# canghaiyang/Erasure_Coding_Test

Measured on AMD Instinct MI355X. Metric: GiB/s device-resident RS encode+decode, RS(10,4) 4 MiB shards, 1/2/4/8 GPU, higher is better.
Workload: dtype u8

## Files before the change

### erasure_coding_test_amd/build.py

```python
from __future__ import annotations

import hashlib
import os
import re
import shutil
import subprocess
import sys

PKG = os.path.dirname(os.path.abspath(__file__))
ROOT = os.path.dirname(PKG)
CSRC = os.path.join(PKG, "csrc")
LIB = os.path.join(PKG, "lib")
OBJ = os.path.join(PKG, "build", "obj")
INCLUDE = os.path.join(ROOT, "include")

ARCH = os.environ.get("ECGPU_ARCH", "gfx950")
HIPCC = os.environ.get("HIPCC", shutil.which("hipcc") or "/opt/rocm/bin/hipcc")
CXX = os.environ.get("CXX", "g++")

HOST_SRCS = ["gf_host.cpp", "matrix_host.cpp", "planner.cpp", "schedule_host.cpp", "capi_host.cpp", "contract_host.cpp", "knobs.cpp",
             "cpu_fallback.cpp", "cpu_exec.cpp"]
HIP_UNITS = [(f, f + ".o", []) for f in ("ecgpu_runtime.hip", "plans.hip", "devices.hip", "contexts.hip",
                                           "host_memory.hip", "dispatch_w8.hip", "dispatch_wide.hip", "accum.hip",
                                           "pipeline.hip", "packets.hip", "scrub.hip")] + [
# ... 2 lines not shown
DROPIN_SRCS = ["jerasure_dropin.cpp", "jerasure_surface.cpp"]

CXXFLAGS = ["-O2", "-std=c++17", "-fPIC", "-Wall", "-Wextra", "-Wno-unused-parameter", f"-I{INCLUDE}", f"-I{CSRC}"]
HIPFLAGS = ["-O3", "-std=c++17", "-fPIC", "-fvisibility=hidden", "-Wall", "-Wextra", "-Wno-unused-parameter", f"--offload-arch={ARCH}", f"-I{INCLUDE}", f"-I{CSRC}",
            "-Wno-unused-result"]


def _run(cmd):
    print("  " + " ".join(cmd), flush=True)
    subprocess.run(cmd, check=True)


def _run_parallel(cmds):
    from concurrent.futures import ThreadPoolExecutor
    if not cmds:
        return
    workers = max(1, min(len(cmds), int(os.environ.get("MAX_JOBS", "0")) or (os.cpu_count() or 1), 8))
    with ThreadPoolExecutor(workers) as ex:
        for f in [ex.submit(_run, c) for c in cmds]:
            f.result()


KERNEL_FAMILIES = {
    "kernels": (["gf_device.hpp", "gf_kernels_w8.hpp", "gf_spec.hip", "gf_spec.hpp", "dispatch_w8.hip"],
                ["ECGPU_CAP", "ECGPU_BLOCKS_PER_CU", "ECGPU_KERNEL", "ECGPU_NT"]),
    "wide": (["gf_device.hpp", "gf_kernels_wide.hpp", "wide_spec.hip", "wide_spec.hpp", "dispatch_wide.hip"],
             ["ECGPU_WIDE", "ECGPU_NIB16", "ECGPU_WIDE_UNITS", "ECGPU_WIDE_PIPE", "ECGPU_WIDE16_BPCU",
              "ECGPU_WIDE16_UNITS"]),
    "packets": (["gf_device.hpp", "gf_kernels_packets.hpp", "packets.hip"], ["ECGPU_PACKET"]),
    "scrub": (["gf_device.hpp", "scrub_kernels.hpp", "scrub_spec.hip", "scrub_spec.hpp", "scrub.hip"],
              ["ECGPU_CAP", "ECGPU_BLOCKS_PER_CU", "ECGPU_SCRUB_LATE"]),
}


def knob_rows(names) -> list:
    with open(os.path.join(CSRC, "knobs.cpp")) as f:
        lines = f.read().splitlines()
    return [ln.strip() for n in names for ln in lines if ln.strip().startswith('{"%s",' % n)]


def _digest(parts, files) -> str:
    h = hashlib.sha256()
    for p in parts:
        h.update(p.encode())
        h.update(b"\0")
    for f in files:
        h.update(os.path.basename(f).encode())
# ... 146 lines not shown
```

### erasure_coding_test_amd/csrc/diag_kernels.hip

```cpp
#include <hip/hip_runtime.h>

#include <cstdlib>

#include "diag_kernels_w8.hpp"

using ecgpu::dev::ApplyArgs;
using ecgpu::dev::u32x4;
using KernelFn = void (*)(ApplyArgs);

namespace {

__device__ __forceinline__ void sink(const ApplyArgs& a, int s, int64_t col, const u32x4& acc) {
  if (acc.x == 0x9E3779B9u && acc.y == 0x7F4A7C15u && acc.z == 0x85EBCA6Bu && acc.w == 0xC2B2AE35u)
    ecgpu::dev::store16(a.dst[int64_t(s) * a.dst_stride], col, acc, 1);
}

template <int K, int R>
__global__ __launch_bounds__(256) void diag_xor_mix(ApplyArgs a) {
  const int64_t col = int64_t(blockIdx.x) * 256 + threadIdx.x;
  if (col >= a.nvec) return;
  const int s = blockIdx.y;
  const uint8_t* const* sp = a.src + int64_t(s) * a.src_stride;
  uint8_t* dp[R];
#pragma unroll
  for (int r = 0; r < R; ++r) dp[r] = a.dst[int64_t(s) * a.dst_stride + r];
  u32x4 x[K];
#pragma unroll
// ... 108 lines not shown
KernelFn pick_mode(int mode) {
  switch (mode) {
    case 0: return &ecgpu::dev::gf_apply_perm<K, R, V, 0>;
    case 1: return &ecgpu::dev::gf_apply_perm<K, R, V, 1>;
    case 2: return &ecgpu::dev::gf_apply_perm<K, R, V, 2>;
    default: return &ecgpu::dev::gf_apply_perm<K, R, V, 3>;
  }
}
template <int K, int R>
KernelFn pick_vec(int vec, int mode) {
  switch (vec) {
    case 1: return pick_mode<K, R, 1>(mode);
    case 2: return pick_mode<K, R, 2>(mode);
    default: return pick_mode<K, R, 4>(mode);
  }
}
}

extern "C" __attribute__((visibility("default"))) int ecgpu_diag_launch(
    int variant, int K, int R, int vec, int mode, const void* qtab, const void* ntab, const void* src_tab,
    void* dst_tab, int stripes, long long size, unsigned long long unit_mask, unsigned long long zero_mask, int nt,
    void* stream, const void* ptab) {
  KernelFn fn = nullptr;
  if (variant == 0) {
    if (K == 10 && R == 4) fn = pick_vec<10, 4>(vec, mode);
    if (K == 10 && R == 1) fn = pick_vec<10, 1>(vec, mode);
  } else if (variant == 1) {
    using ecgpu::dev::diag_copy;
    KernelFn c1[4] = {&diag_copy<1, 0>, &diag_copy<1, 1>, &diag_copy<1, 2>, &diag_copy<1, 3>};
    KernelFn c2[4] = {&diag_copy<2, 0>, &diag_copy<2, 1>, &diag_copy<2, 2>, &diag_copy<2, 3>};
    KernelFn c4[4] = {&diag_copy<4, 0>, &diag_copy<4, 1>, &diag_copy<4, 2>, &diag_copy<4, 3>};
    fn = (vec == 1 ? c1 : vec == 2 ? c2 : c4)[mode & 3];
  } else if (variant == 3) {
    if (K == 10 && R == 4) fn = mode == 3 ? &ecgpu::dev::gf_apply_perm_stream<10, 4, 3>
                                          : &ecgpu::dev::gf_apply_perm_stream<10, 4, 2>;
    if (K == 10 && R == 1) fn = mode == 3 ? &ecgpu::dev::gf_apply_perm_stream<10, 1, 3>
                                          : &ecgpu::dev::gf_apply_perm_stream<10, 1, 2>;
  } else if (variant == 4 || variant == 5) {
    vec = 1;
    if (K == 10 && R == 4)
      fn = mode == 0 ? &ecgpu::dev::gf_apply<10, 4, 0> : mode == 1 ? &ecgpu::dev::gf_apply<10, 4, 1>
                                                        : &ecgpu::dev::gf_apply<10, 4, 3>;
    if (K == 10 && R == 1)
      fn = mode == 4 ? &ecgpu::dev::gf_apply<10, 1, 4> : &ecgpu::dev::gf_apply<10, 1, 0>;
  } else if (variant == 6) {
    vec = 1;
    if (K == 10 && R == 4) fn = &ecgpu::dev::gf_apply_occ8<10, 4, 3>;
    if (K == 10 && R == 1) fn = mode == 4 ? &ecgpu::dev::gf_apply_occ8<10, 1, 4> : &ecgpu::dev::gf_apply_occ8<10, 1, 0>;
  } else if (variant == 7) {
    const bool occ8 = (vec & 2) != 0;
    if (K == 10 && R == 4)
      fn = occ8 ? &ecgpu::dev::gf_apply_occ8<10, 4, 3> : &ecgpu::dev::gf_apply<10, 4, 3>;
    if (K == 10 && R == 1)
      fn = mode == 4 ? (occ8 ? &ecgpu::dev::gf_apply_occ8<10, 1, 4> : &ecgpu::dev::gf_apply<10, 1, 4>)
                     : (occ8 ? &ecgpu::dev::gf_apply_occ8<10, 1, 0> : &ecgpu::dev::gf_apply<10, 1, 0>);
  } else if (variant == 8) {
    if (K == 10 && R == 4)
      fn = vec == 1 ? &ecgpu::dev::gf_apply<10, 4, 3>
                    : vec == 2 ? &ecgpu::dev::gf_apply_vec<10, 4, 3, 2> : &ecgpu::dev::gf_apply_vec<10, 4, 3, 4>;
    if (K == 10 && R == 1)
      fn = vec == 1 ? &ecgpu::dev::gf_apply<10, 1, 4>
                    : vec == 2 ? &ecgpu::dev::gf_apply_vec<10, 1, 4, 2> : &ecgpu::dev::gf_apply_vec<10, 1, 4, 4>;
  } else if (variant == 9) {
    vec = 1;
    if (K == 1 && R == 1) fn = &ecgpu::dev::gf_apply_perm<1, 1, 1, 3>;
    if (K == 2 && R == 2) fn = &ecgpu::dev::gf_apply_perm<2, 2, 1, 3>;
    if (K == 4 && R == 4) fn = &ecgpu::dev::gf_apply_perm<4, 4, 1, 3>;
    if (K == 7 && R == 7) fn = &ecgpu::dev::gf_apply_perm<7, 7, 1, 3>;
    if (K == 10 && R == 4) fn = &ecgpu::dev::gf_apply_perm<10, 4, 1, 3>;
    if (K == 10 && R == 1) fn = &ecgpu::dev::gf_apply_perm<10, 1, 1, 3>;
    if (K == 13 && R == 1) fn = &ecgpu::dev::gf_apply_perm<13, 1, 1, 3>;
    if (K == 4 && R == 1) fn = &ecgpu::dev::gf_apply_perm<4, 1, 1, 3>;
    if (K == 1 && R == 4) fn = &ecgpu::dev::gf_apply_perm<1, 4, 1, 3>;
    if (K == 2 && R == 1) fn = &ecgpu::dev::gf_apply_perm<2, 1, 1, 3>;
  } else if (variant == 10) {
    vec = 1;
    if (K == 10 && R == 4) fn = &ecgpu::dev::gf_apply_2bit<10, 4, 3>;
    if (K == 10 && R == 1) fn = mode == 4 ? &ecgpu::dev::gf_apply_2bit<10, 1, 4> : &ecgpu::dev::gf_apply_2bit<10, 1, 0>;
  } else if (variant == 11) {
    vec = 1;
    if (K == 1) fn = nt ? &diag_read_regs<1, 1> : &diag_read_regs<1, 0>;
    if (K == 4) fn = nt ? &diag_read_regs<4, 1> : &diag_read_regs<4, 0>;
    if (K == 10) fn = nt ? &diag_read_regs<10, 1> : &diag_read_regs<10, 0>;
    if (K == 14) fn = nt ? &diag_read_regs<14, 1> : &diag_read_regs<14, 0>;
  } else if (variant == 13 || variant == 14) {
    using namespace ecgpu::dev;
    const int ntb = vec;
    vec = 1;
#define ECGPU_PICK(KK, RR, UU)                                                                              \
  (variant == 13 ? (ntb == 0 ? &gf_apply<KK, RR, UU, 0> : ntb == 1 ? &gf_apply<KK, RR, UU, 1>         \
                    : ntb == 2 ? &gf_apply<KK, RR, UU, 2> : &gf_apply<KK, RR, UU, 3>)                 \
                 : (ntb == 0 ? &gf_apply_dma<KK, RR, UU, 0> : ntb == 1 ? &gf_apply_dma<KK, RR, UU, 1> \
                    : ntb == 2 ? &gf_apply_dma<KK, RR, UU, 2> : &gf_apply_dma<KK, RR, UU, 3>))
    if (K == 10 && R == 4) fn = mode == 0 ? ECGPU_PICK(10, 4, 0) : ECGPU_PICK(10, 4, 3);
    if (K == 10 && R == 1) fn = mode == 4 ? ECGPU_PICK(10, 1, 4) : ECGPU_PICK(10, 1, 0);
    if (K == 6 && R == 3) fn = ECGPU_PICK(6, 3, 3);
#undef ECGPU_PICK
  } else if (variant == 12) {
    vec = 1;
    if (K == 1) fn = nt ? &diag_read_glds<1, 1> : &diag_read_glds<1, 0>;
    if (K == 4) fn = nt ? &diag_read_glds<4, 1> : &diag_read_glds<4, 0>;
    if (K == 10) fn = nt ? &diag_read_glds<10, 1> : &diag_read_glds<10, 0>;
    if (K == 14) fn = nt ? &diag_read_glds<14, 1> : &diag_read_glds<14, 0>;
  } else if (variant == 15) {
    const int lp = vec;
    vec = 1;
    if (K == 10 && R == 4) fn = pick_pol<10, 4, 3>(lp, mode);
    if (K == 10 && R == 1) fn = pick_pol<10, 1, 4>(lp, mode);
  } else if (variant == 16) {
    vec = 1;
    if (K == 10 && R == 4) fn = &diag_xor_mix<10, 4>;
    if (K == 10 && R == 1) fn = &diag_xor_mix<10, 1>;
    if (K == 6 && R == 3) fn = &diag_xor_mix<6, 3>;
    if (K == 12 && R == 4) fn = &diag_xor_mix<12, 4>;
    if (K == 4 && R == 2) fn = &diag_xor_mix<4, 2>;
  } else if (variant == 2) {
    vec = 1;
    if (K == 10 && R == 4) fn = &ecgpu::dev::gf_apply_lds<10, 4>;
    if (K == 10 && R == 1) fn = &ecgpu::dev::gf_apply_lds<10, 1>;
  }
  if (!fn) return -2;
  ApplyArgs a{};
  a.qtab = static_cast<const ecgpu::dev::u32x4*>(qtab);
  a.ntab = static_cast<const uint8_t*>(ntab);
  a.ptab = static_cast<const uint32_t*>(ptab);
  a.src = static_cast<const uint8_t* const*>(src_tab);
  a.dst = static_cast<uint8_t* const*>(dst_tab);
  a.nvec = size / 16;
  a.size = size;
  a.byte0 = a.nvec * 16;
  a.unit_mask = unit_mask;
  a.zero_mask = zero_mask;
  a.src_stride = variant == 1 ? 1 : K;
  a.dst_stride = variant == 1 ? 1 : R;
  a.row0 = 0;
  a.K = K;
  a.R = R;
  a.nt = nt;
  const long long per_block = 256LL * (variant == 0 || variant == 1 || variant == 8 ? vec : 1);
  dim3 grid(unsigned((a.nvec + per_block - 1) / per_block), unsigned(stripes));
  if (variant == 3) grid = dim3(unsigned(vec), unsigned(stripes));
  if (variant == 7) {
    a.stripe_fast = vec & 1;
    grid = a.stripe_fast ? dim3(unsigned(stripes), unsigned((a.nvec + 255) / 256))
                         : dim3(unsigned((a.nvec + 255) / 256), unsigned(stripes));
  }
  if (variant == 5) {
    a.stripe_fast = 1;
    grid = dim3(unsigned(stripes), unsigned((a.nvec + 255) / 256));
  }
  void* args[] = {&a};
  const char* lds_env = std::getenv("ECGPU_DIAG_LDS");
  const unsigned lds = lds_env ? unsigned(std::atoi(lds_env)) : 0u;
  if (lds > 65536u && lds <= 163840u &&
      hipFuncSetAttribute(reinterpret_cast<const void*>(fn), hipFuncAttributeMaxDynamicSharedMemorySize, int(lds)) !=
          hipSuccess)
    return -3;
  return hipLaunchKernel(reinterpret_cast<const void*>(fn), grid, dim3(256), args, lds,
                         static_cast<hipStream_t>(stream)) == hipSuccess ? 0 : -3;
}
```

### erasure_coding_test_amd/csrc/diag_kernels_w8.hpp

```cpp
#pragma once
#include "gf_kernels.hpp"

namespace ecgpu {
namespace dev {

__device__ __forceinline__ u32x4 load16(const uint8_t* p, int64_t col, int nt) {
  const gu32x4* a = (const gu32x4*)p + col;
  return nt ? __builtin_nontemporal_load(a) : *a;
}

__device__ __forceinline__ void store16(uint8_t* p, int64_t col, const u32x4& v, int nt) {
  gu32x4* a = (gu32x4*)p + col;
  if (nt)
    __builtin_nontemporal_store(v, a);
  else
    *a = v;
}

__device__ __forceinline__ uint32_t mac_word(uint32_t acc, const u32x4& q, uint32_t x) {
  const uint32_t s0 = x & kLo2, s1 = (x >> 2) & kLo2, s2 = (x >> 4) & kLo2, s3 = (x >> 6) & kLo2;
  return xor3(acc, xor3(perm_lookup(q.x, s0), perm_lookup(q.y, s1), perm_lookup(q.z, s2)), perm_lookup(q.w, s3));
}

__device__ __forceinline__ uint32_t mul3(const uint32_t* __restrict__ t, const Sel3& s) {
// ... 202 lines not shown
  if (col >= a.nvec) return;
  const int w = __builtin_amdgcn_readfirstlane(int(threadIdx.x) >> 6);
  const int lane = threadIdx.x & 63;
  const uint8_t* const* sp = a.src + int64_t(s) * a.src_stride;
  const uint8_t* src[K];
#pragma unroll
  for (int j = 0; j < K; ++j) src[j] = sp[j];
  uint8_t* dp[R];
#pragma unroll
  for (int r = 0; r < R; ++r) dp[r] = a.dst[int64_t(s) * a.dst_stride + a.row0 + r];
#pragma unroll
  for (int j = 0; j < K; ++j)
    __builtin_amdgcn_global_load_lds((const __attribute__((address_space(1))) void*)(src[j] + col * 16),
                                     (__attribute__((address_space(3))) void*)&stage[w][j][0], 16, 0,
                                     (NT & 1) ? 2 : 0);
  asm volatile("s_waitcnt vmcnt(0)" ::: "memory");
  u32x4 x[K];
#pragma unroll
  for (int j = 0; j < K; ++j) x[j] = stage[w][j][lane];
  combine_store<K, R, UNITS, (NT >> 1)>(a, x, dp, col);
}

template <int K, int R, int UNITS>
__global__ __launch_bounds__(kBlock, 8) void gf_apply_occ8(ApplyArgs a) {
  gf_apply_body<K, R, UNITS>(a);
}

template <int K, int R, int MODE>
__global__ __launch_bounds__(kBlock) void gf_apply_perm_stream(ApplyArgs a) {
  __shared__ u32x4 lq[R * K];
  for (int i = threadIdx.x; i < R * K; i += kBlock) lq[i] = a.qtab[i];
  __syncthreads();
  const int s = blockIdx.y;
  const int64_t steps_total = (a.nvec + kBlock - 1) / kBlock;
  const int64_t steps_per_block = (steps_total + gridDim.x - 1) / gridDim.x;
  const int64_t step0 = int64_t(blockIdx.x) * steps_per_block;
  const int64_t step_end = step0 + steps_per_block < steps_total ? step0 + steps_per_block : steps_total;
  if (step0 >= step_end) return;
  const uint8_t* const* sp = a.src + int64_t(s) * a.src_stride;
  uint8_t* dp[R];
#pragma unroll
  for (int r = 0; r < R; ++r) dp[r] = a.dst[int64_t(s) * a.dst_stride + a.row0 + r];
  const uint8_t* src[K];
#pragma unroll
  for (int j = 0; j < K; ++j) src[j] = sp[j];

  u32x4 cur[K], nxt[K];
  int64_t col = step0 * kBlock + threadIdx.x;
// ... 57 lines not shown
```

### erasure_coding_test_amd/csrc/dispatch_w8.hip

```cpp
#include <hip/hip_runtime.h>

#include <algorithm>
#include <atomic>
#include <cstdint>
#include <cstring>
#include <mutex>
#include <string>
#include <utility>
#include <vector>

#include "ecgpu.h"
#include "gf_host.hpp"
#include "gf_kernels_w8.hpp"
#include "knobs.hpp"
#include "runtime.hpp"
#include "gf_spec.hpp"

using namespace ecgpu;
using namespace ecgpu::rt;
using dev::ApplyArgs;
using dev::u32x4;

namespace ecgpu {
namespace dev {

static __global__ __launch_bounds__(kBlock) void gf_apply_bytes(ApplyArgs a) {
  const int64_t x = a.byte0 + int64_t(blockIdx.x) * kBlock + threadIdx.x;
  if (x >= a.size) return;
  const int s = blockIdx.y;
  const uint8_t* const* sp = a.src + int64_t(s) * a.src_stride;
  uint8_t* const* dp = a.dst + int64_t(s) * a.dst_stride + a.row0;
  uint32_t acc[kMaxRows] = {0u, 0u, 0u, 0u};
  for (int j = 0; j < a.K; ++j) {
    const uint32_t v = sp[j][x];
    const uint32_t s0 = v & 3u, s1 = (v >> 2) & 3u, s2 = (v >> 4) & 3u, s3 = v >> 6;
    for (int r = 0; r < a.R; ++r) acc[r] ^= gf_mul_perm(a.qtab[r * a.K + j], s0, s1, s2, s3);
  }
// ... 11 lines not shown
    for (int j = 0; j < K; ++j) {
      const bool one = coef[size_t(r0 + r) * K + j] == 1;
      all &= one;
      if (j == 0) col0 &= one;
      if (r == 0) row0 &= one;
    }
  if (all) return 4;
  return (col0 ? 1 : 0) | (row0 ? 2 : 0);
}

KernelFn generic_fn(int R) {
  switch (R) {
    case 1: return &dev::gf_apply_perm_generic<1>;
    case 2: return &dev::gf_apply_perm_generic<2>;
    case 3: return &dev::gf_apply_perm_generic<3>;
    default: return &dev::gf_apply_perm_generic<4>;
  }
}


constexpr int kCapMaxBlocks = 4;
constexpr int kMinWavesPerSimd = 4;
static_assert(kMinWavesPerSimd >= kCapMaxBlocks, "a cap above the register limit is a no-op");
unsigned residency_lds_bytes(int device, int streams, unsigned static_bytes) {
  static std::once_flag once;
  static int per_cu = 0;
  std::call_once(once, [&] {
    if (hipDeviceGetAttribute(&per_cu, hipDeviceAttributeMaxSharedMemoryPerMultiprocessor, device) != hipSuccess)
      per_cu = 0;
  });
  const int fixed = knob(Knob::kBlocksPerCu);
  const int blocks = fixed >= 0 ? fixed : (streams <= 9 ? kCapMaxBlocks : kCapMaxBlocks - 1);
  if (blocks <= 0 || per_cu <= 0) return 0;
  const unsigned total = unsigned(per_cu / blocks) & ~511u;
  const unsigned reserve = static_bytes ? static_bytes + 4096u : 0u;
  if (total <= reserve) return 0;
  const unsigned b = (total - reserve) & (static_bytes ? ~4095u : ~511u);
  return b + static_bytes > unsigned(per_cu / (blocks + 1)) ? b : 0u;
}

bool cap_for(int K, int R, int mul_terms, bool seq) {
  const int v = knob(Knob::kCap);
  return v < 0 ? (seq || 2 * mul_terms <= 5 * (K + R)) : (v != 0);
}

void build_tables(int c, u32x4* q, uint32_t* p3, uint8_t* nib) {
  const auto& T = gf8().mul[c & 0xFF];
  uint32_t w[4];
  for (int p = 0; p < 4; ++p) {
    w[p] = 0;
    for (int e = 0; e < 4; ++e) w[p] |= uint32_t(T[e << (2 * p)]) << (8 * e);
  }
  *q = u32x4{w[0], w[1], w[2], w[3]};
  for (int i = 0; i < dev::kP3Words; ++i) p3[i] = 0;
  for (int e = 0; e < 8; ++e) {
    p3[e >> 2] |= uint32_t(T[e]) << (8 * (e & 3));
    p3[2 + (e >> 2)] |= uint32_t(T[e << 3]) << (8 * (e & 3));
  }
  for (int e = 0; e < 4; ++e) p3[4] |= uint32_t(T[e << 6]) << (8 * e);
  for (int x = 0; x < 16; ++x) {
    nib[x] = T[x];
// ... 10 lines not shown
  for (size_t i = 0; i < n; ++i) build_tables(coefs[i], &q[i], &p3[i * dev::kP3Words], &nib[i * 32]);
  const size_t qb = n * sizeof(u32x4), pb = p3.size() * sizeof(uint32_t), nb = n * 32;
  std::vector<uint8_t> host(qb + pb + nb);
  std::memcpy(host.data(), q.data(), qb);
  std::memcpy(host.data() + qb, p3.data(), pb);
  std::memcpy(host.data() + qb + pb, nib.data(), nb);
  if (int rc = plan_upload_tables(p, std::move(host))) return rc;
  p->d_q = reinterpret_cast<u32x4*>(p->d_tabs);
  p->d_p3 = reinterpret_cast<uint32_t*>(p->d_tabs + qb);
  p->d_nib = p->d_tabs + qb + pb;
  return ECGPU_OK;
}

std::atomic<int64_t> g_engine_launches[2];

int plan_launch(ecgpu_plan* p, hipStream_t stream) {
  if (p->stripes <= 0 || p->size <= 0 || p->rows <= 0) return ECGPU_OK;
  DeviceGuard g(p->device);
  if (int rc = plan_wait_tables(p, stream)) return rc;
  if (p->w != 8) return plan_launch_wide(p, stream);
  const int K = p->nsrc;
  const int64_t nvec = p->aligned ? p->size / 16 : 0;
  const int64_t byte0 = nvec * 16;
  const dim3 block(dev::kBlock);
  for (int r0 = 0; r0 < p->rows; r0 += dev::kMaxRows) {
    const int R = std::min(dev::kMaxRows, p->rows - r0);
    const bool spec = K <= dev::kMaxSpecK;
    int mul_terms = 0;
    for (int r = 0; r < R; ++r)
      for (int j = 0; j < K; ++j) mul_terms += p->coef[size_t(r0 + r) * K + j] > 1u;
    const bool use_lds = p->kind == ECGPU_KERNEL_LDS;
    KernelFn vec_fn = spec ? spec_kernel(use_lds, K, R, unit_variant(p->coef, K, r0, R), p->nt) : generic_fn(R);
    if (spec && nvec > 0) g_engine_launches[use_lds ? 1 : 0].fetch_add(1, std::memory_order_relaxed);
    const int vec = 1;
    const bool cap = cap_for(K, R, mul_terms, spec && !use_lds && R >= dev::kSeqMinRows);
    const unsigned static_lds = use_lds && spec ? unsigned(K) * 32u * 4u : 0u;
    uint64_t unit = 0, zero = 0;
    if (spec)
      for (int r = 0; r < R; ++r)
        for (int j = 0; j < K; ++j) {
          const uint32_t c = p->coef[size_t(r0 + r) * K + j];
          if (c == 1) unit |= uint64_t(1) << (r * K + j);
          if (c == 0) zero |= uint64_t(1) << (r * K + j);
        }
    for (int s0 = 0; s0 < p->stripes; s0 += dev::kMaxGridY) {
      const int ns = std::min(dev::kMaxGridY, p->stripes - s0);
      ApplyArgs a{};
      a.qtab = p->d_q + size_t(r0) * K;
      a.ptab = p->d_p3 + size_t(r0) * K * dev::kP3Words;
      a.ntab = p->d_nib + size_t(r0) * K * 32;
      a.src = p->d_src + size_t(s0) * K;
      a.dst = p->d_dst + size_t(s0) * p->rows;
      a.nvec = nvec;
      a.size = p->size;
      a.byte0 = byte0;
      a.src_stride = K;
      a.dst_stride = p->rows;
      a.row0 = r0;
      a.K = K;
      a.R = R;
      a.nt = p->nt;
      a.unit_mask = unit;
      a.zero_mask = zero;
      if (nvec > 0) {
        const int64_t per_block = int64_t(dev::kBlock) * vec;
        const dim3 grid(unsigned((nvec + per_block - 1) / per_block), unsigned(ns));
        const unsigned lds = cap ? residency_lds_bytes(p->device, K + R, static_lds) : 0u;
        ECGPU_HIP(launch(vec_fn, grid, block, a, stream, lds));
      }
      if (byte0 < p->size) {
        const dim3 grid(unsigned((p->size - byte0 + dev::kBlock - 1) / dev::kBlock), unsigned(ns));
        ECGPU_HIP(launch(&dev::gf_apply_bytes, grid, block, a, stream));
      }
    }
  }
  return ECGPU_OK;
}

ECGPU_RT_END

extern "C" ECGPU_API int64_t ecgpu_engine_launches(int kind) {
  return kind == 0 || kind == 1 ? ecgpu::rt::g_engine_launches[kind].load(std::memory_order_relaxed) : -1;
}
```

### erasure_coding_test_amd/csrc/gf_kernels_w8.hpp

```cpp
#pragma once
#include <hip/hip_runtime.h>
#include <stdint.h>

#include "gf_device.hpp"

namespace ecgpu {
namespace dev {

template <int K, int R, int UNITS>
__device__ __forceinline__ void combine(const ApplyArgs& a, const u32x4 (&x)[K], u32x4 (&acc)[R]) {
  combine3<K, R, UNITS>((const kconst_u32*)a.ptab, x, acc);
}

template <int K, int R, int UNITS, int NTS>
__device__ __forceinline__ void combine_store(const ApplyArgs& a, const u32x4 (&x)[K], uint8_t* const (&dp)[R],
                                              int64_t col) {
  u32x4 acc[R];
  combine<K, R, UNITS>(a, x, acc);
#pragma unroll
  for (int r = 0; r < R; ++r) store16t<NTS>(dp[r], col, acc[r]);
}

constexpr int kSeqMinRows = 3;
template <int K>
constexpr int load_window() { return K <= 10 ? 6 : K; }

template <int K, int R, int UNITS, int NT = 3>
__device__ __forceinline__ void gf_apply_body(const ApplyArgs& a) {
  const unsigned cblk = a.stripe_fast ? blockIdx.y : blockIdx.x;
  const int s = a.stripe_fast ? blockIdx.x : blockIdx.y;
  const int64_t col0 = int64_t(cblk) * kBlock + threadIdx.x;
  if (col0 >= a.nvec) return;
  const uint8_t* const* sp = a.src + int64_t(s) * a.src_stride;
  uint8_t* dp[R];
#pragma unroll
  for (int r = 0; r < R; ++r) dp[r] = a.dst[int64_t(s) * a.dst_stride + a.row0 + r];

  if constexpr (R >= kSeqMinRows) {
    constexpr int G = load_window<K>();
    const kconst_u32* ptab = (const kconst_u32*)a.ptab;
    u32x4 x[K];
#pragma unroll
    for (int j = 0; j < K && j < G; ++j) x[j] = load16t<NT & 1>(sp[j], col0);
    Xacc xa[R][4];
#pragma unroll
    for (int j = 0; j < K; ++j) {
      __builtin_amdgcn_sched_barrier(0);
      if (j + G < K) x[j + G] = load16t<NT & 1>(sp[j + G], col0);
      Sel3 sl[4];
#pragma unroll
      for (int c = 0; c < 4; ++c) sl[c] = sel3(x[j][c]);
#pragma unroll
      for (int r = 0; r < R; ++r) {
        if (is_unit<UNITS>(r, j)) {
#pragma unroll
          for (int c = 0; c < 4; ++c) xa[r][c].add(x[j][c]);
        } else {
          const kconst_u32* t = ptab + (r * K + j) * kP3Words;
#pragma unroll
          for (int c = 0; c < 4; ++c) mac3(xa[r][c], t, sl[c]);
        }
      }
    }
    __builtin_amdgcn_sched_barrier(0);
#pragma unroll
    for (int r = 0; r < R; ++r) {
      u32x4 o;
#pragma unroll
      for (int c = 0; c < 4; ++c) o[c] = xa[r][c].value();
      store16t<(NT >> 1)>(dp[r], col0, o);
    }
  } else {
    u32x4 x[K];
#pragma unroll
    for (int j = 0; j < K; ++j) x[j] = load16t<NT & 1>(sp[j], col0);
    combine_store<K, R, UNITS, (NT >> 1)>(a, x, dp, col0);
  }
}

template <int K, int R, int UNITS, int NT = 3>
__global__ __launch_bounds__(kBlock) void gf_apply(ApplyArgs a) {
  gf_apply_body<K, R, UNITS, NT>(a);
}

template <int K, int R, int UNITS>
__device__ __forceinline__ void inl_column(const uint8_t* const (&sp)[K], uint8_t* const (&dp)[R],
                                           const kconst_u32* t, int64_t col) {
  u32x4 x[K];
#pragma unroll
  for (int j = 0; j < K; ++j) x[j] = load16t<1>(sp[j], col);
  u32x4 acc[R];
  combine3<K, R, UNITS>(t, x, acc);
#pragma unroll
  for (int r = 0; r < R; ++r) store16t<1>(dp[r], col, acc[r]);
}

template <int K, int R, int UNITS, bool ZC>
__global__ __launch_bounds__(kBlock) void gf_apply_inl(InlineArgs a) {
  const kconst_u32* ptab = (const kconst_u32*)a.ptab;
  if (int(blockIdx.x) < a.nblk_vec) {
    const uint8_t* sp[K];
#pragma unroll
    for (int j = 0; j < K; ++j) sp[j] = a.src[j];
    uint8_t* dp[R];
// ... 159 lines not shown
```

### erasure_coding_test_amd/csrc/gf_spec.hip

```cpp
#include <hip/hip_runtime.h>

#include "gf_kernels_w8.hpp"
#include "gf_spec.hpp"

#ifndef ECGPU_SPEC_R
#error "build with -DECGPU_SPEC_R=<1..4>"
#endif

namespace ecgpu {
namespace {

constexpr int kR = ECGPU_SPEC_R;
constexpr int kUnitVariants[5] = {dev::kUnitNone, dev::kUnitCol0, dev::kUnitRow0, dev::kUnitCol0 | dev::kUnitRow0,
                                  dev::kUnitAll};

template <int K, int U, int STORE>
constexpr SpecKernelFn apply_fn() { return &dev::gf_apply<K, kR, kUnitVariants[U], 1 | (STORE << 1)>; }

template <int K, int S>
struct Pol {
  static constexpr SpecKernelFn apply[5] = {apply_fn<K, 0, S>(), apply_fn<K, 1, S>(), apply_fn<K, 2, S>(),
                                            apply_fn<K, 3, S>(), apply_fn<K, 4, S>()};
};

template <int K, int U, bool ZC>
constexpr InlineKernelFn inl_fn() { return &dev::gf_apply_inl<K, kR, kUnitVariants[U], ZC>; }

template <int K>
struct Row {
  static constexpr InlineKernelFn inl[2][5] = {
      {inl_fn<K, 0, false>(), inl_fn<K, 1, false>(), inl_fn<K, 2, false>(), inl_fn<K, 3, false>(), inl_fn<K, 4, false>()},
      {inl_fn<K, 0, true>(), inl_fn<K, 1, true>(), inl_fn<K, 2, true>(), inl_fn<K, 3, true>(), inl_fn<K, 4, true>()}};
  static constexpr const SpecKernelFn* apply[kStorePolicies] = {Pol<K, 0>::apply, Pol<K, 1>::apply};
  static constexpr SpecKernelFn lds = &dev::gf_apply_lds<K, kR>;
};

template <int... Ks>
SpecKernelFn pick(bool lds, int K, int u, int store_pol) {
  SpecKernelFn out = nullptr;
  ((K == Ks ? (out = lds ? Row<Ks>::lds : Row<Ks>::apply[store_pol][u], 0) : 0), ...);
  return out;
}

template <int... Ks>
InlineKernelFn pick_inl(int K, int u, bool zc) {
  InlineKernelFn out = nullptr;
  ((K == Ks ? (out = Row<Ks>::inl[zc ? 1 : 0][u], 0) : 0), ...);
  return out;
}

}

#define ECGPU_CAT2(a, b) a##b
#define ECGPU_CAT(a, b) ECGPU_CAT2(a, b)
SpecKernelFn ECGPU_CAT(spec_kernel_r, ECGPU_SPEC_R)(bool lds, int K, int unit_variant, int store_pol) {
  if (unit_variant < 0 || unit_variant > 4 || store_pol < 0 || store_pol >= kStorePolicies) return nullptr;
  return pick<1, 2, 3, 4, 5, 6, 7, 8, 9, 10, 11, 12, 13, 14, 15, 16>(lds, K, unit_variant, store_pol);
}

InlineKernelFn ECGPU_CAT(inline_kernel_r, ECGPU_SPEC_R)(int K, int unit_variant, bool zc) {
  if (unit_variant < 0 || unit_variant > 4) return nullptr;
  return pick_inl<1, 2, 3, 4, 5, 6, 7, 8, 9, 10, 11, 12, 13, 14, 15, 16>(K, unit_variant, zc);
}

}
```

### erasure_coding_test_amd/csrc/gf_spec.hpp

```cpp
#pragma once
#include "gf_device.hpp"

namespace ecgpu {

using SpecKernelFn = void (*)(dev::ApplyArgs);
using InlineKernelFn = void (*)(dev::InlineArgs);
constexpr int kStorePolicies = 2;

SpecKernelFn spec_kernel_r1(bool lds, int K, int unit_variant, int store_pol);
SpecKernelFn spec_kernel_r2(bool lds, int K, int unit_variant, int store_pol);
SpecKernelFn spec_kernel_r3(bool lds, int K, int unit_variant, int store_pol);
SpecKernelFn spec_kernel_r4(bool lds, int K, int unit_variant, int store_pol);

InlineKernelFn inline_kernel_r1(int K, int unit_variant, bool zc);
InlineKernelFn inline_kernel_r2(int K, int unit_variant, bool zc);
InlineKernelFn inline_kernel_r3(int K, int unit_variant, bool zc);
InlineKernelFn inline_kernel_r4(int K, int unit_variant, bool zc);

inline InlineKernelFn inline_kernel(int K, int R, int unit_variant, bool zc) {
  switch (R) {
    case 1: return inline_kernel_r1(K, unit_variant, zc);
    case 2: return inline_kernel_r2(K, unit_variant, zc);
    case 3: return inline_kernel_r3(K, unit_variant, zc);
    case 4: return inline_kernel_r4(K, unit_variant, zc);
    default: return nullptr;
  }
}

inline SpecKernelFn spec_kernel(bool lds, int K, int R, int unit_variant, int store_pol) {
  switch (R) {
    case 1: return spec_kernel_r1(lds, K, unit_variant, store_pol);
    case 2: return spec_kernel_r2(lds, K, unit_variant, store_pol);
    case 3: return spec_kernel_r3(lds, K, unit_variant, store_pol);
    case 4: return spec_kernel_r4(lds, K, unit_variant, store_pol);
    default: return nullptr;
  }
}

}
```

### erasure_coding_test_amd/csrc/runtime.hpp

```cpp
#pragma once
#include <hip/hip_runtime.h>

#include <algorithm>
#include <cstdint>
#include <list>
#include <memory>
#include <mutex>
#include <string>
#include <utility>
#include <vector>

#include "ecgpu.h"
#include "gf_device.hpp"
#include "gf_spec.hpp"
#include "knobs.hpp"
#include "planner.hpp"

#define ECGPU_RT_BEGIN \
  namespace ecgpu {    \
  namespace __attribute__((visibility("hidden"))) rt {
#define ECGPU_RT_END \
  }                  \
  }

// ... 54 lines not shown
  }
  ~DeviceGuard() {
    int cur = -1;
    if (prev >= 0 && hipGetDevice(&cur) == hipSuccess && cur != prev) (void)hipSetDevice(prev);
  }
};

int current_device();
int visible_devices();
int forced_device();
std::shared_ptr<const std::vector<int>> device_list();
int host_call_device();
int call_device(const std::vector<void*>& a, const std::vector<void*>& b);

using KernelFn = void (*)(ecgpu::dev::ApplyArgs);

inline hipError_t launch(KernelFn fn, dim3 grid, dim3 block, ecgpu::dev::ApplyArgs& a, hipStream_t s,
                         unsigned lds_bytes = 0) {
  void* args[] = {&a};
  return hipLaunchKernel(reinterpret_cast<const void*>(fn), grid, block, args, lds_bytes, s);
}

int unit_variant(const std::vector<uint32_t>& coef, int K, int r0, int R);
unsigned residency_lds_bytes(int device, int streams, unsigned static_bytes = 0);
bool cap_for(int K, int R, int mul_terms, bool seq = false);

inline int clamp_store_policy(int nt) { return std::min(kStorePolicies - 1, std::max(0, nt)); }
void plan_free(ecgpu_plan* p);
int plan_upload_tables(ecgpu_plan* p, std::vector<uint8_t>&& host);
int plan_wait_tables(ecgpu_plan* p, hipStream_t stream);
int plan_sync_tables(ecgpu_plan* p);
int plan_init_w8(ecgpu_plan* p, const int* coefs);
int plan_init_wide(ecgpu_plan* p, const int* coefs);
int plan_launch_wide(ecgpu_plan* p, hipStream_t stream);
int plan_init(ecgpu_plan* p, int rows, int nsrc, const int* coefs, int device, int w = 8);
int plan_bind(ecgpu_plan* p, int stripes, const uint8_t* const* src, uint8_t* const* dst, int64_t size,
              hipStream_t stream, bool keep_alive = false);
int plan_launch(ecgpu_plan* p, hipStream_t stream);

struct PlanKey {
  int rows, nsrc, w, kind, nt;
  std::vector<uint32_t> coef;
  bool operator==(const PlanKey& o) const {
    return rows == o.rows && nsrc == o.nsrc && w == o.w && kind == o.kind && nt == o.nt && coef == o.coef;
  }
};

// ... 43 lines not shown
```

Measured before the change: 4840.

## Use one-wave workgroups for RS(10,4) apply on shards up to 4 MiB

```diff
diff --git a/erasure_coding_test_amd/build.py b/erasure_coding_test_amd/build.py
--- a/erasure_coding_test_amd/build.py
+++ b/erasure_coding_test_amd/build.py
@@ -48,7 +48,7 @@
 
 
 KERNEL_FAMILIES = {
-    "kernels": (["gf_device.hpp", "gf_kernels_w8.hpp", "gf_spec.hip", "gf_spec.hpp", "dispatch_w8.hip"],
+    "kernels": (["gf_device.hpp", "gf_kernels_w8.hpp", "gf_spec.hip", "gf_spec.hpp", "dispatch_w8.hip", "residency_w8.hpp"],
                 ["ECGPU_CAP", "ECGPU_BLOCKS_PER_CU", "ECGPU_KERNEL", "ECGPU_NT"]),
     "wide": (["gf_device.hpp", "gf_kernels_wide.hpp", "wide_spec.hip", "wide_spec.hpp", "dispatch_wide.hip"],
              ["ECGPU_WIDE", "ECGPU_NIB16", "ECGPU_WIDE_UNITS", "ECGPU_WIDE_PIPE", "ECGPU_WIDE16_BPCU",
diff --git a/erasure_coding_test_amd/csrc/diag_kernels.hip b/erasure_coding_test_amd/csrc/diag_kernels.hip
--- a/erasure_coding_test_amd/csrc/diag_kernels.hip
+++ b/erasure_coding_test_amd/csrc/diag_kernels.hip
@@ -3,6 +3,7 @@
 #include <cstdlib>
 
 #include "diag_kernels_w8.hpp"
+#include "residency_w8.hpp"
 
 using ecgpu::dev::ApplyArgs;
 using ecgpu::dev::u32x4;
@@ -157,6 +158,9 @@
     void* dst_tab, int stripes, long long size, unsigned long long unit_mask, unsigned long long zero_mask, int nt,
     void* stream, const void* ptab) {
   KernelFn fn = nullptr;
+  int lanes = 256;
+#define PROD(KK, RR, UU, NN) (lanes = ecgpu::dev::apply_block<KK, RR, UU, NN>(), &ecgpu::dev::gf_apply<KK, RR, UU, NN>)
+#define OCC8(KK, RR, UU) (lanes = ecgpu::dev::apply_block<KK, RR, UU, 3>(), &ecgpu::dev::gf_apply_occ8<KK, RR, UU>)
   if (variant == 0) {
     if (K == 10 && R == 4) fn = pick_vec<10, 4>(vec, mode);
     if (K == 10 && R == 1) fn = pick_vec<10, 1>(vec, mode);
@@ -174,27 +178,27 @@
   } else if (variant == 4 || variant == 5) {
     vec = 1;
     if (K == 10 && R == 4)
-      fn = mode == 0 ? &ecgpu::dev::gf_apply<10, 4, 0> : mode == 1 ? &ecgpu::dev::gf_apply<10, 4, 1>
-                                                        : &ecgpu::dev::gf_apply<10, 4, 3>;
+      fn = mode == 0 ? PROD(10, 4, 0, 3) : mode == 1 ? PROD(10, 4, 1, 3)
+                                                        : PROD(10, 4, 3, 3);
     if (K == 10 && R == 1)
-      fn = mode == 4 ? &ecgpu::dev::gf_apply<10, 1, 4> : &ecgpu::dev::gf_apply<10, 1, 0>;
+      fn = mode == 4 ? PROD(10, 1, 4, 3) : PROD(10, 1, 0, 3);
   } else if (variant == 6) {
     vec = 1;
-    if (K == 10 && R == 4) fn = &ecgpu::dev::gf_apply_occ8<10, 4, 3>;
-    if (K == 10 && R == 1) fn = mode == 4 ? &ecgpu::dev::gf_apply_occ8<10, 1, 4> : &ecgpu::dev::gf_apply_occ8<10, 1, 0>;
+    if (K == 10 && R == 4) fn = OCC8(10, 4, 3);
+    if (K == 10 && R == 1) fn = mode == 4 ? OCC8(10, 1, 4) : OCC8(10, 1, 0);
   } else if (variant == 7) {
     const bool occ8 = (vec & 2) != 0;
     if (K == 10 && R == 4)
-      fn = occ8 ? &ecgpu::dev::gf_apply_occ8<10, 4, 3> : &ecgpu::dev::gf_apply<10, 4, 3>;
+      fn = occ8 ? OCC8(10, 4, 3) : PROD(10, 4, 3, 3);
     if (K == 10 && R == 1)
-      fn = mode == 4 ? (occ8 ? &ecgpu::dev::gf_apply_occ8<10, 1, 4> : &ecgpu::dev::gf_apply<10, 1, 4>)
-                     : (occ8 ? &ecgpu::dev::gf_apply_occ8<10, 1, 0> : &ecgpu::dev::gf_apply<10, 1, 0>);
+      fn = mode == 4 ? (occ8 ? OCC8(10, 1, 4) : PROD(10, 1, 4, 3))
+                     : (occ8 ? OCC8(10, 1, 0) : PROD(10, 1, 0, 3));
   } else if (variant == 8) {
     if (K == 10 && R == 4)
-      fn = vec == 1 ? &ecgpu::dev::gf_apply<10, 4, 3>
+      fn = vec == 1 ? PROD(10, 4, 3, 3)
                     : vec == 2 ? &ecgpu::dev::gf_apply_vec<10, 4, 3, 2> : &ecgpu::dev::gf_apply_vec<10, 4, 3, 4>;
     if (K == 10 && R == 1)
-      fn = vec == 1 ? &ecgpu::dev::gf_apply<10, 1, 4>
+      fn = vec == 1 ? PROD(10, 1, 4, 3)
                     : vec == 2 ? &ecgpu::dev::gf_apply_vec<10, 1, 4, 2> : &ecgpu::dev::gf_apply_vec<10, 1, 4, 4>;
   } else if (variant == 9) {
     vec = 1;
@@ -223,8 +227,8 @@
     const int ntb = vec;
     vec = 1;
 #define ECGPU_PICK(KK, RR, UU)                                                                              \
-  (variant == 13 ? (ntb == 0 ? &gf_apply<KK, RR, UU, 0> : ntb == 1 ? &gf_apply<KK, RR, UU, 1>         \
-                    : ntb == 2 ? &gf_apply<KK, RR, UU, 2> : &gf_apply<KK, RR, UU, 3>)                 \
+  (variant == 13 ? (ntb == 0 ? PROD(KK, RR, UU, 0) : ntb == 1 ? PROD(KK, RR, UU, 1)         \
+                    : ntb == 2 ? PROD(KK, RR, UU, 2) : PROD(KK, RR, UU, 3))                 \
                  : (ntb == 0 ? &gf_apply_dma<KK, RR, UU, 0> : ntb == 1 ? &gf_apply_dma<KK, RR, UU, 1> \
                     : ntb == 2 ? &gf_apply_dma<KK, RR, UU, 2> : &gf_apply_dma<KK, RR, UU, 3>))
     if (K == 10 && R == 4) fn = mode == 0 ? ECGPU_PICK(10, 4, 0) : ECGPU_PICK(10, 4, 3);
@@ -254,6 +258,8 @@
     if (K == 10 && R == 4) fn = &ecgpu::dev::gf_apply_lds<10, 4>;
     if (K == 10 && R == 1) fn = &ecgpu::dev::gf_apply_lds<10, 1>;
   }
+#undef PROD
+#undef OCC8
   if (!fn) return -2;
   ApplyArgs a{};
   a.qtab = static_cast<const ecgpu::dev::u32x4*>(qtab);
@@ -272,17 +278,17 @@
   a.K = K;
   a.R = R;
   a.nt = nt;
-  const long long per_block = 256LL * (variant == 0 || variant == 1 || variant == 8 ? vec : 1);
+  const long long per_block = (long long)lanes * (variant == 0 || variant == 1 || variant == 8 ? vec : 1);
   dim3 grid(unsigned((a.nvec + per_block - 1) / per_block), unsigned(stripes));
   if (variant == 3) grid = dim3(unsigned(vec), unsigned(stripes));
   if (variant == 7) {
     a.stripe_fast = vec & 1;
-    grid = a.stripe_fast ? dim3(unsigned(stripes), unsigned((a.nvec + 255) / 256))
-                         : dim3(unsigned((a.nvec + 255) / 256), unsigned(stripes));
+    grid = a.stripe_fast ? dim3(unsigned(stripes), unsigned((a.nvec + lanes - 1) / lanes))
+                         : dim3(unsigned((a.nvec + lanes - 1) / lanes), unsigned(stripes));
   }
   if (variant == 5) {
     a.stripe_fast = 1;
-    grid = dim3(unsigned(stripes), unsigned((a.nvec + 255) / 256));
+    grid = dim3(unsigned(stripes), unsigned((a.nvec + lanes - 1) / lanes));
   }
   void* args[] = {&a};
   const char* lds_env = std::getenv("ECGPU_DIAG_LDS");
@@ -291,6 +297,32 @@
       hipFuncSetAttribute(reinterpret_cast<const void*>(fn), hipFuncAttributeMaxDynamicSharedMemorySize, int(lds)) !=
           hipSuccess)
     return -3;
-  return hipLaunchKernel(reinterpret_cast<const void*>(fn), grid, dim3(256), args, lds,
+  return hipLaunchKernel(reinterpret_cast<const void*>(fn), grid, dim3(unsigned(lanes)), args, lds,
                          static_cast<hipStream_t>(stream)) == hipSuccess ? 0 : -3;
 }
+
+extern "C" __attribute__((visibility("default"))) int ecgpu_diag_apply_residency(
+    int K, int R, int units, int store_nt, int big, int waves_per_cu, int* lanes, unsigned* dyn_lds,
+    int* workgroups_per_cu) {
+  using namespace ecgpu::dev;
+  KernelFn fn = nullptr;
+  int block = 0;
+#define ECGPU_PICK1(KK, RR, UU, NN) (block = apply_block<KK, RR, UU, NN>(), &gf_apply<KK, RR, UU, NN>)
+#define ECGPU_PICK(KK, RR, UU)                                                                              \
+  (big && has_one_wave_form<KK, RR, UU>() ? (store_nt ? ECGPU_PICK1(KK, RR, UU, 7) : ECGPU_PICK1(KK, RR, UU, 5)) \
+                                           : (store_nt ? ECGPU_PICK1(KK, RR, UU, 3) : ECGPU_PICK1(KK, RR, UU, 1)))
+  if (K == 10 && R == 4 && units == 3) fn = ECGPU_PICK(10, 4, 3);
+  if (K == 10 && R == 4 && units == 0) fn = ECGPU_PICK(10, 4, 0);
+  if (K == 10 && R == 1 && units == 4) fn = ECGPU_PICK(10, 1, 4);
+#undef ECGPU_PICK
+#undef ECGPU_PICK1
+  if (!fn || !lanes || !dyn_lds || !workgroups_per_cu) return -2;
+  int device = 0, per_cu = 0;
+  if (hipGetDevice(&device) != hipSuccess ||
+      hipDeviceGetAttribute(&per_cu, hipDeviceAttributeMaxSharedMemoryPerMultiprocessor, device) != hipSuccess)
+    return -3;
+  *lanes = block;
+  *dyn_lds = ecgpu::residency_lds_for(per_cu, ecgpu::residency_workgroups(waves_per_cu, block), 0u);
+  return hipOccupancyMaxActiveBlocksPerMultiprocessor(workgroups_per_cu, reinterpret_cast<const void*>(fn), block,
+                                                      *dyn_lds) == hipSuccess ? 0 : -3;
+}
diff --git a/erasure_coding_test_amd/csrc/diag_kernels_w8.hpp b/erasure_coding_test_amd/csrc/diag_kernels_w8.hpp
--- a/erasure_coding_test_amd/csrc/diag_kernels_w8.hpp
+++ b/erasure_coding_test_amd/csrc/diag_kernels_w8.hpp
@@ -248,8 +248,13 @@
 }
 
 template <int K, int R, int UNITS>
-__global__ __launch_bounds__(kBlock, 8) void gf_apply_occ8(ApplyArgs a) {
+__global__ __launch_bounds__((apply_block<K, R, UNITS, 3>()), 8) void gf_apply_occ8(ApplyArgs a) {
   gf_apply_body<K, R, UNITS>(a);
+}
+
+template <int K, int R, int UNITS, int BS>
+__global__ __launch_bounds__(BS) void gf_apply_wg(ApplyArgs a) {
+  gf_apply_body<K, R, UNITS, 3, BS>(a);
 }
 
 template <int K, int R, int MODE>
diff --git a/erasure_coding_test_amd/csrc/dispatch_w8.hip b/erasure_coding_test_amd/csrc/dispatch_w8.hip
--- a/erasure_coding_test_amd/csrc/dispatch_w8.hip
+++ b/erasure_coding_test_amd/csrc/dispatch_w8.hip
@@ -13,6 +13,7 @@
 #include "gf_host.hpp"
 #include "gf_kernels_w8.hpp"
 #include "knobs.hpp"
+#include "residency_w8.hpp"
 #include "runtime.hpp"
 #include "gf_spec.hpp"
 
@@ -70,21 +71,24 @@
 constexpr int kCapMaxBlocks = 4;
 constexpr int kMinWavesPerSimd = 4;
 static_assert(kMinWavesPerSimd >= kCapMaxBlocks, "a cap above the register limit is a no-op");
-unsigned residency_lds_bytes(int device, int streams, unsigned static_bytes) {
+constexpr int kWavesPerBlock = dev::kBlock / kLanesPerWave;
+constexpr int kCapWavesOneWave = 10;
+static_assert(kCapWavesOneWave <= kMinWavesPerSimd * kWavesPerBlock, "a cap above the register limit is a no-op");
+int residency_waves_per_cu(int streams, int lanes) {
+  const int fixed = knob(Knob::kBlocksPerCu);
+  if (fixed >= 0) return fixed * kWavesPerBlock;
+  if (lanes < dev::kBlock) return kCapWavesOneWave;
+  return (streams <= 9 ? kCapMaxBlocks : kCapMaxBlocks - 1) * kWavesPerBlock;
+}
+
+unsigned residency_lds_bytes(int device, int streams, unsigned static_bytes, int lanes) {
   static std::once_flag once;
   static int per_cu = 0;
   std::call_once(once, [&] {
     if (hipDeviceGetAttribute(&per_cu, hipDeviceAttributeMaxSharedMemoryPerMultiprocessor, device) != hipSuccess)
       per_cu = 0;
   });
-  const int fixed = knob(Knob::kBlocksPerCu);
-  const int blocks = fixed >= 0 ? fixed : (streams <= 9 ? kCapMaxBlocks : kCapMaxBlocks - 1);
-  if (blocks <= 0 || per_cu <= 0) return 0;
-  const unsigned total = unsigned(per_cu / blocks) & ~511u;
-  const unsigned reserve = static_bytes ? static_bytes + 4096u : 0u;
-  if (total <= reserve) return 0;
-  const unsigned b = (total - reserve) & (static_bytes ? ~4095u : ~511u);
-  return b + static_bytes > unsigned(per_cu / (blocks + 1)) ? b : 0u;
+  return residency_lds_for(per_cu, residency_workgroups(residency_waves_per_cu(streams, lanes), lanes), static_bytes);
 }
 
 bool cap_for(int K, int R, int mul_terms, bool seq) {
@@ -141,7 +145,6 @@
   const int K = p->nsrc;
   const int64_t nvec = p->aligned ? p->size / 16 : 0;
   const int64_t byte0 = nvec * 16;
-  const dim3 block(dev::kBlock);
   for (int r0 = 0; r0 < p->rows; r0 += dev::kMaxRows) {
     const int R = std::min(dev::kMaxRows, p->rows - r0);
     const bool spec = K <= dev::kMaxSpecK;
@@ -149,9 +152,11 @@
     for (int r = 0; r < R; ++r)
       for (int j = 0; j < K; ++j) mul_terms += p->coef[size_t(r0 + r) * K + j] > 1u;
     const bool use_lds = p->kind == ECGPU_KERNEL_LDS;
-    KernelFn vec_fn = spec ? spec_kernel(use_lds, K, R, unit_variant(p->coef, K, r0, R), p->nt) : generic_fn(R);
+    const bool big = p->size > dev::kOneWaveMaxShard;
+    const SpecKernel vec_k = spec ? spec_kernel(use_lds, K, R, unit_variant(p->coef, K, r0, R), p->nt, big)
+                                  : SpecKernel{generic_fn(R), dev::kBlock};
+    if (!vec_k.fn || vec_k.block <= 0) return ECGPU_ERR_ARG;
     if (spec && nvec > 0) g_engine_launches[use_lds ? 1 : 0].fetch_add(1, std::memory_order_relaxed);
-    const int vec = 1;
     const bool cap = cap_for(K, R, mul_terms, spec && !use_lds && R >= dev::kSeqMinRows);
     const unsigned static_lds = use_lds && spec ? unsigned(K) * 32u * 4u : 0u;
     uint64_t unit = 0, zero = 0;
@@ -182,14 +187,14 @@
       a.unit_mask = unit;
       a.zero_mask = zero;
       if (nvec > 0) {
-        const int64_t per_block = int64_t(dev::kBlock) * vec;
+        const int64_t per_block = vec_k.block;
         const dim3 grid(unsigned((nvec + per_block - 1) / per_block), unsigned(ns));
-        const unsigned lds = cap ? residency_lds_bytes(p->device, K + R, static_lds) : 0u;
-        ECGPU_HIP(launch(vec_fn, grid, block, a, stream, lds));
+        const unsigned lds = cap ? residency_lds_bytes(p->device, K + R, static_lds, vec_k.block) : 0u;
+        ECGPU_HIP(launch(vec_k.fn, grid, dim3(unsigned(vec_k.block)), a, stream, lds));
       }
       if (byte0 < p->size) {
         const dim3 grid(unsigned((p->size - byte0 + dev::kBlock - 1) / dev::kBlock), unsigned(ns));
-        ECGPU_HIP(launch(&dev::gf_apply_bytes, grid, block, a, stream));
+        ECGPU_HIP(launch(&dev::gf_apply_bytes, grid, dim3(dev::kBlock), a, stream));
       }
     }
   }
diff --git a/erasure_coding_test_amd/csrc/gf_kernels_w8.hpp b/erasure_coding_test_amd/csrc/gf_kernels_w8.hpp
--- a/erasure_coding_test_amd/csrc/gf_kernels_w8.hpp
+++ b/erasure_coding_test_amd/csrc/gf_kernels_w8.hpp
@@ -25,11 +25,20 @@
 template <int K>
 constexpr int load_window() { return K <= 10 ? 6 : K; }
 
-template <int K, int R, int UNITS, int NT = 3>
+constexpr int kNt256Lanes = 4;
+constexpr int64_t kOneWaveMaxShard = int64_t(4) << 20;
+template <int K, int R, int UNITS>
+constexpr bool has_one_wave_form() {
+  return UNITS == (kUnitCol0 | kUnitRow0) && ((K == 10 && R == 4) || (K == 6 && R == 3));
+}
+template <int K, int R, int UNITS, int NT>
+constexpr int apply_block() { return has_one_wave_form<K, R, UNITS>() && !(NT & kNt256Lanes) ? 64 : kBlock; }
+
+template <int K, int R, int UNITS, int NT = 3, int BS = apply_block<K, R, UNITS, NT>()>
 __device__ __forceinline__ void gf_apply_body(const ApplyArgs& a) {
   const unsigned cblk = a.stripe_fast ? blockIdx.y : blockIdx.x;
   const int s = a.stripe_fast ? blockIdx.x : blockIdx.y;
-  const int64_t col0 = int64_t(cblk) * kBlock + threadIdx.x;
+  const int64_t col0 = int64_t(cblk) * BS + threadIdx.x;
   if (col0 >= a.nvec) return;
   const uint8_t* const* sp = a.src + int64_t(s) * a.src_stride;
   uint8_t* dp[R];
@@ -68,18 +77,18 @@
       u32x4 o;
 #pragma unroll
       for (int c = 0; c < 4; ++c) o[c] = xa[r][c].value();
-      store16t<(NT >> 1)>(dp[r], col0, o);
+      store16t<((NT >> 1) & 1)>(dp[r], col0, o);
     }
   } else {
     u32x4 x[K];
 #pragma unroll
     for (int j = 0; j < K; ++j) x[j] = load16t<NT & 1>(sp[j], col0);
-    combine_store<K, R, UNITS, (NT >> 1)>(a, x, dp, col0);
+    combine_store<K, R, UNITS, ((NT >> 1) & 1)>(a, x, dp, col0);
   }
 }
 
 template <int K, int R, int UNITS, int NT = 3>
-__global__ __launch_bounds__(kBlock) void gf_apply(ApplyArgs a) {
+__global__ __launch_bounds__((apply_block<K, R, UNITS, NT>())) void gf_apply(ApplyArgs a) {
   gf_apply_body<K, R, UNITS, NT>(a);
 }
 
diff --git a/erasure_coding_test_amd/csrc/gf_spec.hip b/erasure_coding_test_amd/csrc/gf_spec.hip
--- a/erasure_coding_test_amd/csrc/gf_spec.hip
+++ b/erasure_coding_test_amd/csrc/gf_spec.hip
@@ -14,13 +14,16 @@
 constexpr int kUnitVariants[5] = {dev::kUnitNone, dev::kUnitCol0, dev::kUnitRow0, dev::kUnitCol0 | dev::kUnitRow0,
                                   dev::kUnitAll};
 
-template <int K, int U, int STORE>
-constexpr SpecKernelFn apply_fn() { return &dev::gf_apply<K, kR, kUnitVariants[U], 1 | (STORE << 1)>; }
+template <int K, int U, int STORE, bool BIG>
+constexpr SpecKernel apply_fn() {
+  constexpr int NT = 1 | (STORE << 1) | (BIG && dev::has_one_wave_form<K, kR, kUnitVariants[U]>() ? dev::kNt256Lanes : 0);
+  return SpecKernel{&dev::gf_apply<K, kR, kUnitVariants[U], NT>, dev::apply_block<K, kR, kUnitVariants[U], NT>()};
+}
 
-template <int K, int S>
+template <int K, int S, bool BIG>
 struct Pol {
-  static constexpr SpecKernelFn apply[5] = {apply_fn<K, 0, S>(), apply_fn<K, 1, S>(), apply_fn<K, 2, S>(),
-                                            apply_fn<K, 3, S>(), apply_fn<K, 4, S>()};
+  static constexpr SpecKernel apply[5] = {apply_fn<K, 0, S, BIG>(), apply_fn<K, 1, S, BIG>(), apply_fn<K, 2, S, BIG>(),
+                                          apply_fn<K, 3, S, BIG>(), apply_fn<K, 4, S, BIG>()};
 };
 
 template <int K, int U, bool ZC>
@@ -31,14 +34,15 @@
   static constexpr InlineKernelFn inl[2][5] = {
       {inl_fn<K, 0, false>(), inl_fn<K, 1, false>(), inl_fn<K, 2, false>(), inl_fn<K, 3, false>(), inl_fn<K, 4, false>()},
       {inl_fn<K, 0, true>(), inl_fn<K, 1, true>(), inl_fn<K, 2, true>(), inl_fn<K, 3, true>(), inl_fn<K, 4, true>()}};
-  static constexpr const SpecKernelFn* apply[kStorePolicies] = {Pol<K, 0>::apply, Pol<K, 1>::apply};
+  static constexpr const SpecKernel* apply[2][kStorePolicies] = {{Pol<K, 0, false>::apply, Pol<K, 1, false>::apply},
+                                                                 {Pol<K, 0, true>::apply, Pol<K, 1, true>::apply}};
   static constexpr SpecKernelFn lds = &dev::gf_apply_lds<K, kR>;
 };
 
 template <int... Ks>
-SpecKernelFn pick(bool lds, int K, int u, int store_pol) {
-  SpecKernelFn out = nullptr;
-  ((K == Ks ? (out = lds ? Row<Ks>::lds : Row<Ks>::apply[store_pol][u], 0) : 0), ...);
+SpecKernel pick(bool lds, int K, int u, int store_pol, bool big) {
+  SpecKernel out;
+  ((K == Ks ? (out = lds ? SpecKernel{Row<Ks>::lds, dev::kBlock} : Row<Ks>::apply[big ? 1 : 0][store_pol][u], 0) : 0), ...);
   return out;
 }
 
@@ -53,9 +57,9 @@
 
 #define ECGPU_CAT2(a, b) a##b
 #define ECGPU_CAT(a, b) ECGPU_CAT2(a, b)
-SpecKernelFn ECGPU_CAT(spec_kernel_r, ECGPU_SPEC_R)(bool lds, int K, int unit_variant, int store_pol) {
-  if (unit_variant < 0 || unit_variant > 4 || store_pol < 0 || store_pol >= kStorePolicies) return nullptr;
-  return pick<1, 2, 3, 4, 5, 6, 7, 8, 9, 10, 11, 12, 13, 14, 15, 16>(lds, K, unit_variant, store_pol);
+SpecKernel ECGPU_CAT(spec_kernel_r, ECGPU_SPEC_R)(bool lds, int K, int unit_variant, int store_pol, bool big) {
+  if (unit_variant < 0 || unit_variant > 4 || store_pol < 0 || store_pol >= kStorePolicies) return {};
+  return pick<1, 2, 3, 4, 5, 6, 7, 8, 9, 10, 11, 12, 13, 14, 15, 16>(lds, K, unit_variant, store_pol, big);
 }
 
 InlineKernelFn ECGPU_CAT(inline_kernel_r, ECGPU_SPEC_R)(int K, int unit_variant, bool zc) {
diff --git a/erasure_coding_test_amd/csrc/gf_spec.hpp b/erasure_coding_test_amd/csrc/gf_spec.hpp
--- a/erasure_coding_test_amd/csrc/gf_spec.hpp
+++ b/erasure_coding_test_amd/csrc/gf_spec.hpp
@@ -4,13 +4,17 @@
 namespace ecgpu {
 
 using SpecKernelFn = void (*)(dev::ApplyArgs);
+struct SpecKernel {
+  SpecKernelFn fn = nullptr;
+  int block = 0;
+};
 using InlineKernelFn = void (*)(dev::InlineArgs);
 constexpr int kStorePolicies = 2;
 
-SpecKernelFn spec_kernel_r1(bool lds, int K, int unit_variant, int store_pol);
-SpecKernelFn spec_kernel_r2(bool lds, int K, int unit_variant, int store_pol);
-SpecKernelFn spec_kernel_r3(bool lds, int K, int unit_variant, int store_pol);
-SpecKernelFn spec_kernel_r4(bool lds, int K, int unit_variant, int store_pol);
+SpecKernel spec_kernel_r1(bool lds, int K, int unit_variant, int store_pol, bool big);
+SpecKernel spec_kernel_r2(bool lds, int K, int unit_variant, int store_pol, bool big);
+SpecKernel spec_kernel_r3(bool lds, int K, int unit_variant, int store_pol, bool big);
+SpecKernel spec_kernel_r4(bool lds, int K, int unit_variant, int store_pol, bool big);
 
 InlineKernelFn inline_kernel_r1(int K, int unit_variant, bool zc);
 InlineKernelFn inline_kernel_r2(int K, int unit_variant, bool zc);
@@ -27,13 +31,13 @@
   }
 }
 
-inline SpecKernelFn spec_kernel(bool lds, int K, int R, int unit_variant, int store_pol) {
+inline SpecKernel spec_kernel(bool lds, int K, int R, int unit_variant, int store_pol, bool big) {
   switch (R) {
-    case 1: return spec_kernel_r1(lds, K, unit_variant, store_pol);
-    case 2: return spec_kernel_r2(lds, K, unit_variant, store_pol);
-    case 3: return spec_kernel_r3(lds, K, unit_variant, store_pol);
-    case 4: return spec_kernel_r4(lds, K, unit_variant, store_pol);
-    default: return nullptr;
+    case 1: return spec_kernel_r1(lds, K, unit_variant, store_pol, big);
+    case 2: return spec_kernel_r2(lds, K, unit_variant, store_pol, big);
+    case 3: return spec_kernel_r3(lds, K, unit_variant, store_pol, big);
+    case 4: return spec_kernel_r4(lds, K, unit_variant, store_pol, big);
+    default: return {};
   }
 }
 
diff --git a/erasure_coding_test_amd/csrc/residency_w8.hpp b/erasure_coding_test_amd/csrc/residency_w8.hpp
--- /dev/null
+++ b/erasure_coding_test_amd/csrc/residency_w8.hpp
@@ -0,0 +1,20 @@
+#pragma once
+
+namespace ecgpu {
+
+constexpr int kLanesPerWave = 64;
+
+inline int residency_workgroups(int waves_per_cu, int lanes) {
+  return waves_per_cu / ((lanes + kLanesPerWave - 1) / kLanesPerWave);
+}
+
+inline unsigned residency_lds_for(int lds_per_cu, int workgroups, unsigned static_bytes) {
+  if (workgroups <= 0 || lds_per_cu <= 0) return 0;
+  const unsigned total = unsigned(lds_per_cu / workgroups) & ~511u;
+  const unsigned reserve = static_bytes ? static_bytes + 4096u : 0u;
+  if (total <= reserve) return 0;
+  const unsigned b = (total - reserve) & (static_bytes ? ~4095u : ~511u);
+  return b + static_bytes > unsigned(lds_per_cu / (workgroups + 1)) ? b : 0u;
+}
+
+}
diff --git a/erasure_coding_test_amd/csrc/runtime.hpp b/erasure_coding_test_amd/csrc/runtime.hpp
--- a/erasure_coding_test_amd/csrc/runtime.hpp
+++ b/erasure_coding_test_amd/csrc/runtime.hpp
@@ -100,7 +100,8 @@
 }
 
 int unit_variant(const std::vector<uint32_t>& coef, int K, int r0, int R);
-unsigned residency_lds_bytes(int device, int streams, unsigned static_bytes = 0);
+unsigned residency_lds_bytes(int device, int streams, unsigned static_bytes = 0, int lanes = ecgpu::dev::kBlock);
+int residency_waves_per_cu(int streams, int lanes);
 bool cap_for(int K, int R, int mul_terms, bool seq = false);
 
 inline int clamp_store_policy(int nt) { return std::min(kStorePolicies - 1, std::max(0, nt)); }
```

Result: faster. 4897 (median of 6 runs) (+1.2%).
